# evalf/nutils

Measured on AMD Instinct MI355X. Metric: elements assembled/sec (global stiffness K), higher is better.
Workload: dtype f64; 1 GPU; 3D Poisson stiffness, 128^3 structured hex, p=1, 2x2x2 Gauss, iso geometry (BASELINE.json configs[1]); nelems_per_gpu=2097152, nnz_per_gpu=57066625, kernel=k_p1hex_skew<16,16,false,false>, parallelism=single GPU, launch=hipGraph replay (20 steps per graph), settle_steps=600

## Files before the change

nutils_amd/csrc/nh_p1hex_element.inc:

```
        double X[2][2][2][3];
        double un[8];
#pragma unroll
        for (int a = 0; a < 2; ++a)
#pragma unroll
          for (int bb = 0; bb < 2; ++bb)
#pragma unroll
            for (int c = 0; c < 2; ++c) {
              const double *src = NH_P1HEX_VERT(a, bb, c);
              X[a][bb][c][0] = src[0];
              X[a][bb][c][1] = src[1];
              X[a][bb][c][2] = src[2];
              un[a * 4 + bb * 2 + c] = VEC ? src[VW - 1] : 0.;
            }
#define NH_P1HEX_ELEM (((i64)gi * p.n1 + gj) * p.n2 + gk)
        double qs[8];
#pragma unroll
        for (int q = 0; q < 8; ++q) qs[q] = 1.;
        if (COEF && p.qscale) {
          const double *src = p.qscale + NH_P1HEX_ELEM * 8;
#pragma unroll
          for (int q = 0; q < 8; ++q) qs[q] = src[q];
        }
        constexpr bool hasm = MASS;
        double qm[8];
#pragma unroll
        for (int q = 0; q < 8; ++q) qm[q] = 1.;
        if (MASS && COEF && p.qmass) {
          const double *src = p.qmass + NH_P1HEX_ELEM * 8;
#pragma unroll
          for (int q = 0; q < 8; ++q) qm[q] = src[q];
        }
        double *const pl[2] = {acc + slot_of(gi) + (ej * VK + ek) * NS, acc + slot_of(gi + 1) + (ej * VK + ek) * NS};
#define NH_P1HEX_SLOT(a0, a1, a2, b0, b1, b2) (pl[a0] + ((a1) * VK + (a2)) * NS + ((b0) - (a0)) * 9 + ((b1) - (a1)) * 3 + ((b2) - (a2)))
        if constexpr (VEC) {
          double r[8];
#define NH_P1HEX_QS(q) qs[q]
#define NH_P1HEX_QM(q) qm[q]
#include "nh_p1hex_apply.inc"
#undef NH_P1HEX_QS
#undef NH_P1HEX_QM
#pragma unroll
          for (int a = 0; a < 8; ++a) atomicAdd(NH_P1HEX_SLOT(a >> 2, (a >> 1) & 1, a & 1, a >> 2, (a >> 1) & 1, a & 1), r[a]);
        } else {
        double R0[3][3], R1[3][3], R2[3][3], W01[2][2][3], W02[2][2][3], W12[2][2][3], Mm[3][3][3];
#define NH_P1HEX_QS(q) qs[q]
#define NH_P1HEX_QM(q) qm[q]
#include "nh_p1hex_math.inc"
#undef NH_P1HEX_QS
#undef NH_P1HEX_QM
        auto entry = [&](int a, int bb) {
          const int a0 = a >> 2, a1 = (a >> 1) & 1, a2 = a & 1;
          const int b0 = bb >> 2, b1 = (bb >> 1) & 1, b2 = bb & 1;
          const int p0 = a0 + b0, p1 = a1 + b1, p2 = a2 + b2;
          const double s00 = (a0 == b0) ? 1. : -1., s11 = (a1 == b1) ? 1. : -1., s22 = (a2 == b2) ? 1. : -1.;
          const double s01 = (a0 == b1) ? 1. : -1., s10 = (b0 == a1) ? 1. : -1.;
          const double s02 = (a0 == b2) ? 1. : -1., s20 = (b0 == a2) ? 1. : -1.;
          const double s12 = (a1 == b2) ? 1. : -1., s21 = (b1 == a2) ? 1. : -1.;
          double k = s00 * R0[p1][p2] + s11 * R1[p0][p2] + s22 * R2[p0][p1] + s01 * W01[b0][a1][p2] + s10 * W01[a0][b1][p2]
                   + s02 * W02[b0][a2][p1] + s20 * W02[a0][b2][p1] + s12 * W12[b1][a2][p0] + s21 * W12[a1][b2][p0];
          if (hasm) k += Mm[p0][p1][p2];
          return k;
        };
        {
#pragma unroll
          for (int a = 0; a < 8; ++a) {
            const int a0 = a >> 2, a1 = (a >> 1) & 1, a2 = a & 1;
#pragma unroll
            for (int bb = a; bb < 8; ++bb) {
              const int b0 = bb >> 2, b1 = (bb >> 1) & 1, b2 = bb & 1;
              const double k = entry(a, bb);
              double *const dst = NH_P1HEX_SLOT(a0, a1, a2, b0, b1, b2);
              if (!(DEBUG(p) & 1)) atomicAdd(dst, k);
              else if (k == 1.2345e300) dst[0] = 1.;
            }
          }
        }
        }
#undef NH_P1HEX_ELEM
#undef NH_P1HEX_SLOT
```

nutils_amd/csrc/nh_p1hex_math.inc:

```
{
  const double (&n)[2][2] = p.n;
  const double (&c)[3][2] = p.c;
  double J0[2][2][3], J1[2][2][3], J2[2][2][3];
#pragma unroll
  for (int d = 0; d < 3; ++d) {
    double e0[2][2], e1[2][2], e2[2][2];
#pragma unroll
    for (int x = 0; x < 2; ++x)
#pragma unroll
      for (int y = 0; y < 2; ++y) {
        e0[x][y] = X[1][x][y][d] - X[0][x][y][d];
        e1[x][y] = X[x][1][y][d] - X[x][0][y][d];
        e2[x][y] = X[x][y][1][d] - X[x][y][0][d];
      }
    double t0[2][2], t1[2][2], t2[2][2];
#pragma unroll
    for (int y = 0; y < 2; ++y) {
      const double d0 = e0[1][y] - e0[0][y], d1 = e1[1][y] - e1[0][y], d2 = e2[1][y] - e2[0][y];
#pragma unroll
      for (int q1 = 0; q1 < 2; ++q1) {
        t0[q1][y] = fma(n[1][q1], d0, e0[0][y]);
        t1[q1][y] = fma(n[1][q1], d1, e1[0][y]);
        t2[q1][y] = fma(n[1][q1], d2, e2[0][y]);
      }
    }
#pragma unroll
    for (int q1 = 0; q1 < 2; ++q1) {
      const double d0 = t0[q1][1] - t0[q1][0], d1 = t1[q1][1] - t1[q1][0], d2 = t2[q1][1] - t2[q1][0];
#pragma unroll
      for (int q2 = 0; q2 < 2; ++q2) {
        J0[q1][q2][d] = fma(n[1][q2], d0, t0[q1][0]);
        J1[q1][q2][d] = fma(n[1][q2], d1, t1[q1][0]);
        J2[q1][q2][d] = fma(n[1][q2], d2, t2[q1][0]);
      }
    }
  }
  double D0[2][2], D1[2][2], D2[2][2], M01[2][2][2], M02[2][2][2], M12[2][2][2], Dm[2][2][2];
#pragma unroll
  for (int qa = 0; qa < 2; ++qa)
#pragma unroll
    for (int qb = 0; qb < 2; ++qb)
#pragma unroll
      for (int qc = 0; qc < 2; ++qc) {
        const double *c0 = J0[qb][qc], *c1 = J1[qa][qc], *c2 = J2[qa][qb];
        double A[3][3];
        A[0][0] = c1[1] * c2[2] - c1[2] * c2[1];
        A[0][1] = c1[2] * c2[0] - c1[0] * c2[2];
        A[0][2] = c1[0] * c2[1] - c1[1] * c2[0];
        A[1][0] = c2[1] * c0[2] - c2[2] * c0[1];
        A[1][1] = c2[2] * c0[0] - c2[0] * c0[2];
        A[1][2] = c2[0] * c0[1] - c2[1] * c0[0];
        A[2][0] = c0[1] * c1[2] - c0[2] * c1[1];
        A[2][1] = c0[2] * c1[0] - c0[0] * c1[2];
        A[2][2] = c0[0] * c1[1] - c0[1] * c1[0];
        const double det = c0[0] * A[0][0] + c0[1] * A[0][1] + c0[2] * A[0][2];
        const double sc = p.wk[qa][qb][qc] * NH_P1HEX_QS(qa * 4 + qb * 2 + qc) * fast_rcp(fabs(det));
        const double m00 = sc * (A[0][0] * A[0][0] + A[0][1] * A[0][1] + A[0][2] * A[0][2]);
        const double m11 = sc * (A[1][0] * A[1][0] + A[1][1] * A[1][1] + A[1][2] * A[1][2]);
        const double m22 = sc * (A[2][0] * A[2][0] + A[2][1] * A[2][1] + A[2][2] * A[2][2]);
        M01[qa][qb][qc] = sc * (A[0][0] * A[1][0] + A[0][1] * A[1][1] + A[0][2] * A[1][2]);
        M02[qa][qb][qc] = sc * (A[0][0] * A[2][0] + A[0][1] * A[2][1] + A[0][2] * A[2][2]);
        M12[qa][qb][qc] = sc * (A[1][0] * A[2][0] + A[1][1] * A[2][1] + A[1][2] * A[2][2]);
        D0[qb][qc] = qa ? D0[qb][qc] + m00 : m00;
        D1[qa][qc] = qb ? D1[qa][qc] + m11 : m11;
        D2[qa][qb] = qc ? D2[qa][qb] + m22 : m22;
        if (hasm) Dm[qa][qb][qc] = p.wm[qa][qb][qc] * NH_P1HEX_QM(qa * 4 + qb * 2 + qc) * fabs(det);
      }
  {
    double U[2][3];
#pragma unroll
    for (int x = 0; x < 2; ++x)
#pragma unroll
      for (int pp = 0; pp < 3; ++pp) U[x][pp] = c[pp][0] * D0[x][0] + c[pp][1] * D0[x][1];
#pragma unroll
    for (int p1 = 0; p1 < 3; ++p1)
#pragma unroll
      for (int p2 = 0; p2 < 3; ++p2) R0[p1][p2] = c[p1][0] * U[0][p2] + c[p1][1] * U[1][p2];
#pragma unroll
    for (int x = 0; x < 2; ++x)
#pragma unroll
      for (int pp = 0; pp < 3; ++pp) U[x][pp] = c[pp][0] * D1[x][0] + c[pp][1] * D1[x][1];
#pragma unroll
    for (int p0 = 0; p0 < 3; ++p0)
#pragma unroll
      for (int p2 = 0; p2 < 3; ++p2) R1[p0][p2] = c[p0][0] * U[0][p2] + c[p0][1] * U[1][p2];
#pragma unroll
    for (int x = 0; x < 2; ++x)
#pragma unroll
      for (int pp = 0; pp < 3; ++pp) U[x][pp] = c[pp][0] * D2[x][0] + c[pp][1] * D2[x][1];
#pragma unroll
    for (int p0 = 0; p0 < 3; ++p0)
#pragma unroll
      for (int p1 = 0; p1 < 3; ++p1) R2[p0][p1] = c[p0][0] * U[0][p1] + c[p0][1] * U[1][p1];
  }
  {
    double V[2][2][2], V2[2][2][2];
#pragma unroll
    for (int b0 = 0; b0 < 2; ++b0)
#pragma unroll
      for (int be = 0; be < 2; ++be)
#pragma unroll
        for (int ga = 0; ga < 2; ++ga) V[b0][be][ga] = n[b0][0] * M01[0][be][ga] + n[b0][1] * M01[1][be][ga];
#pragma unroll
    for (int b0 = 0; b0 < 2; ++b0)
#pragma unroll
      for (int a1 = 0; a1 < 2; ++a1)
#pragma unroll
        for (int ga = 0; ga < 2; ++ga) V2[b0][a1][ga] = n[a1][0] * V[b0][0][ga] + n[a1][1] * V[b0][1][ga];
#pragma unroll
    for (int b0 = 0; b0 < 2; ++b0)
#pragma unroll
      for (int a1 = 0; a1 < 2; ++a1)
#pragma unroll
        for (int pp = 0; pp < 3; ++pp) W01[b0][a1][pp] = c[pp][0] * V2[b0][a1][0] + c[pp][1] * V2[b0][a1][1];
#pragma unroll
    for (int b0 = 0; b0 < 2; ++b0)
#pragma unroll
      for (int be = 0; be < 2; ++be)
#pragma unroll
        for (int ga = 0; ga < 2; ++ga) V[b0][be][ga] = n[b0][0] * M02[0][be][ga] + n[b0][1] * M02[1][be][ga];
#pragma unroll
    for (int b0 = 0; b0 < 2; ++b0)
#pragma unroll
      for (int a2 = 0; a2 < 2; ++a2)
#pragma unroll
        for (int be = 0; be < 2; ++be) V2[b0][a2][be] = n[a2][0] * V[b0][be][0] + n[a2][1] * V[b0][be][1];
#pragma unroll
    for (int b0 = 0; b0 < 2; ++b0)
#pragma unroll
      for (int a2 = 0; a2 < 2; ++a2)
#pragma unroll
        for (int pp = 0; pp < 3; ++pp) W02[b0][a2][pp] = c[pp][0] * V2[b0][a2][0] + c[pp][1] * V2[b0][a2][1];
#pragma unroll
    for (int b1 = 0; b1 < 2; ++b1)
#pragma unroll
      for (int al = 0; al < 2; ++al)
#pragma unroll
        for (int ga = 0; ga < 2; ++ga) V[b1][al][ga] = n[b1][0] * M12[al][0][ga] + n[b1][1] * M12[al][1][ga];
#pragma unroll
    for (int b1 = 0; b1 < 2; ++b1)
#pragma unroll
      for (int a2 = 0; a2 < 2; ++a2)
#pragma unroll
        for (int al = 0; al < 2; ++al) V2[b1][a2][al] = n[a2][0] * V[b1][al][0] + n[a2][1] * V[b1][al][1];
#pragma unroll
    for (int b1 = 0; b1 < 2; ++b1)
#pragma unroll
      for (int a2 = 0; a2 < 2; ++a2)
#pragma unroll
        for (int pp = 0; pp < 3; ++pp) W12[b1][a2][pp] = c[pp][0] * V2[b1][a2][0] + c[pp][1] * V2[b1][a2][1];
  }
  if (hasm) {
    double t1[2][2][3], t2[2][3][3];
#pragma unroll
    for (int qa = 0; qa < 2; ++qa)
#pragma unroll
      for (int qb = 0; qb < 2; ++qb)
#pragma unroll
        for (int p2 = 0; p2 < 3; ++p2) t1[qa][qb][p2] = c[p2][0] * Dm[qa][qb][0] + c[p2][1] * Dm[qa][qb][1];
#pragma unroll
    for (int qa = 0; qa < 2; ++qa)
#pragma unroll
      for (int p1 = 0; p1 < 3; ++p1)
#pragma unroll
        for (int p2 = 0; p2 < 3; ++p2) t2[qa][p1][p2] = c[p1][0] * t1[qa][0][p2] + c[p1][1] * t1[qa][1][p2];
#pragma unroll
    for (int p0 = 0; p0 < 3; ++p0)
#pragma unroll
      for (int p1 = 0; p1 < 3; ++p1)
#pragma unroll
        for (int p2 = 0; p2 < 3; ++p2) Mm[p0][p1][p2] = c[p0][0] * t2[0][p1][p2] + c[p0][1] * t2[1][p1][p2];
  }
}
```

Baseline: 11.91 billion elements/s.

## Factor P1 hex entry assembly, simplify Jacobian interpolation, inline reciprocal refinement

The per-entry loop that summed nine signed terms for each of the 36 upper-triangle stiffness entries is replaced by a staged evaluation per p0 slice. It precomputes shared sums S, P, Y01 and Y02 so common subexpressions are reused across entries. The Jacobian setup is rewritten as a trilinear coefficient form with fewer subtractions and FMAs. The reciprocal of the determinant now uses the hardware rcp estimate plus one inlined second-order refinement instead of fast_rcp. The aim is fewer FP64 instructions per element, at the cost of more intricate index logic and slightly different rounding.

```diff
diff --git a/nutils_amd/csrc/nh_p1hex_element.inc b/nutils_amd/csrc/nh_p1hex_element.inc
--- a/nutils_amd/csrc/nh_p1hex_element.inc
+++ b/nutils_amd/csrc/nh_p1hex_element.inc
@@ -48,33 +48,12 @@
 #include "nh_p1hex_math.inc"
 #undef NH_P1HEX_QS
 #undef NH_P1HEX_QM
-        auto entry = [&](int a, int bb) {
-          const int a0 = a >> 2, a1 = (a >> 1) & 1, a2 = a & 1;
-          const int b0 = bb >> 2, b1 = (bb >> 1) & 1, b2 = bb & 1;
-          const int p0 = a0 + b0, p1 = a1 + b1, p2 = a2 + b2;
-          const double s00 = (a0 == b0) ? 1. : -1., s11 = (a1 == b1) ? 1. : -1., s22 = (a2 == b2) ? 1. : -1.;
-          const double s01 = (a0 == b1) ? 1. : -1., s10 = (b0 == a1) ? 1. : -1.;
-          const double s02 = (a0 == b2) ? 1. : -1., s20 = (b0 == a2) ? 1. : -1.;
-          const double s12 = (a1 == b2) ? 1. : -1., s21 = (b1 == a2) ? 1. : -1.;
-          double k = s00 * R0[p1][p2] + s11 * R1[p0][p2] + s22 * R2[p0][p1] + s01 * W01[b0][a1][p2] + s10 * W01[a0][b1][p2]
-                   + s02 * W02[b0][a2][p1] + s20 * W02[a0][b2][p1] + s12 * W12[b1][a2][p0] + s21 * W12[a1][b2][p0];
-          if (hasm) k += Mm[p0][p1][p2];
-          return k;
-        };
-        {
-#pragma unroll
-          for (int a = 0; a < 8; ++a) {
-            const int a0 = a >> 2, a1 = (a >> 1) & 1, a2 = a & 1;
-#pragma unroll
-            for (int bb = a; bb < 8; ++bb) {
-              const int b0 = bb >> 2, b1 = (bb >> 1) & 1, b2 = bb & 1;
-              const double k = entry(a, bb);
-              double *const dst = NH_P1HEX_SLOT(a0, a1, a2, b0, b1, b2);
-              if (!(DEBUG(p) & 1)) atomicAdd(dst, k);
-              else if (k == 1.2345e300) dst[0] = 1.;
-            }
-          }
-        }
+#define NH_P1HEX_ENTRY(a0, a1, a2, b0, b1, b2, k) { \
+          double *const dst = NH_P1HEX_SLOT(a0, a1, a2, b0, b1, b2); \
+          if (!(DEBUG(p) & 1)) atomicAdd(dst, k); \
+          else if (k == 1.2345e300) dst[0] = 1.; }
+#include "nh_p1hex_entries.inc"
+#undef NH_P1HEX_ENTRY
         }
 #undef NH_P1HEX_ELEM
 #undef NH_P1HEX_SLOT
diff --git a/nutils_amd/csrc/nh_p1hex_entries.inc b/nutils_amd/csrc/nh_p1hex_entries.inc
--- /dev/null
+++ b/nutils_amd/csrc/nh_p1hex_entries.inc
@@ -0,0 +1,44 @@
+#pragma unroll
+for (int p0 = 0; p0 < 3; ++p0) {
+  const int a0 = p0 == 2, b0 = p0 >= 1;
+  double S[3][3], P[4][4], Y01[2][2][3], Y02[2][2][3];
+#pragma unroll
+  for (int p1 = 0; p1 < 3; ++p1)
+#pragma unroll
+    for (int p2 = 0; p2 < 3; ++p2) {
+      double s = (p0 == 1 ? -R0[p1][p2] : R0[p1][p2]) + (p1 == 1 ? -R1[p0][p2] : R1[p0][p2]);
+      s += p2 == 1 ? -R2[p0][p1] : R2[p0][p1];
+      if (hasm) s += Mm[p0][p1][p2];
+      S[p1][p2] = s;
+    }
+#pragma unroll
+  for (int u = 0; u < 4; ++u)
+#pragma unroll
+    for (int v = u; v < 4; ++v) {
+      const int x = u >> 1, y = u & 1, z = v >> 1, w = v & 1;
+      if (u == v) P[u][v] = fma(x == y ? 2. : -2., W12[x][y][p0], S[2 * x][2 * y]);
+      else P[u][v] = (S[x + z][y + w] + (x == w ? W12[z][y][p0] : -W12[z][y][p0])) + (z == y ? W12[x][w][p0] : -W12[x][w][p0]);
+    }
+#pragma unroll
+  for (int y = 0; y < 2; ++y)
+#pragma unroll
+    for (int w = (a0 == b0 ? y + 1 : 0); w < 2; ++w)
+#pragma unroll
+      for (int pp = 0; pp < 3; ++pp) {
+        const int x = a0, z = b0;
+        Y01[y][w][pp] = (x == w ? W01[z][y][pp] : -W01[z][y][pp]) + (z == y ? W01[x][w][pp] : -W01[x][w][pp]);
+        Y02[y][w][pp] = (x == w ? W02[z][y][pp] : -W02[z][y][pp]) + (z == y ? W02[x][w][pp] : -W02[x][w][pp]);
+      }
+#pragma unroll
+  for (int u = 0; u < 4; ++u)
+#pragma unroll
+    for (int v = (a0 == b0 ? u : 0); v < 4; ++v) {
+      const int a1 = u >> 1, a2 = u & 1, b1 = v >> 1, b2 = v & 1, p1 = a1 + b1, p2 = a2 + b2;
+      double k = P[u < v ? u : v][u < v ? v : u];
+      if (a0 == b0 && a1 == b1) k = fma(a0 == a1 ? 2. : -2., W01[a0][a1][p2], k);
+      else k += Y01[a1][b1][p2];
+      if (a0 == b0 && a2 == b2) k = fma(a0 == a2 ? 2. : -2., W02[a0][a2][p1], k);
+      else k += Y02[a0 == b0 && a2 > b2 ? b2 : a2][a0 == b0 && a2 > b2 ? a2 : b2][p1];
+      NH_P1HEX_ENTRY(a0, a1, a2, b0, b1, b2, k)
+    }
+}
diff --git a/nutils_amd/csrc/nh_p1hex_math.inc b/nutils_amd/csrc/nh_p1hex_math.inc
--- a/nutils_amd/csrc/nh_p1hex_math.inc
+++ b/nutils_amd/csrc/nh_p1hex_math.inc
@@ -1,39 +1,33 @@
+#ifndef NH_P1HEX_RCP_EST
+#define NH_P1HEX_RCP_EST(d) __builtin_amdgcn_rcp(d)
+#endif
 {
   const double (&n)[2][2] = p.n;
   const double (&c)[3][2] = p.c;
   double J0[2][2][3], J1[2][2][3], J2[2][2][3];
 #pragma unroll
   for (int d = 0; d < 3; ++d) {
-    double e0[2][2], e1[2][2], e2[2][2];
+    const double a0 = X[1][0][0][d] - X[0][0][0][d], a1 = X[0][1][0][d] - X[0][0][0][d], a2 = X[0][0][1][d] - X[0][0][0][d];
+    const double f02 = X[1][0][1][d] - X[0][0][1][d];
+    const double a01 = (X[1][1][0][d] - X[0][1][0][d]) - a0, a02 = f02 - a0, a12 = (X[0][1][1][d] - X[0][0][1][d]) - a1;
+    const double a012 = ((X[1][1][1][d] - X[0][1][1][d]) - f02) - a01;
+    double u0[2], v0[2], u1[2], u2[2], v12[2];
 #pragma unroll
-    for (int x = 0; x < 2; ++x)
-#pragma unroll
-      for (int y = 0; y < 2; ++y) {
-        e0[x][y] = X[1][x][y][d] - X[0][x][y][d];
-        e1[x][y] = X[x][1][y][d] - X[x][0][y][d];
-        e2[x][y] = X[x][y][1][d] - X[x][y][0][d];
-      }
-    double t0[2][2], t1[2][2], t2[2][2];
-#pragma unroll
-    for (int y = 0; y < 2; ++y) {
-      const double d0 = e0[1][y] - e0[0][y], d1 = e1[1][y] - e1[0][y], d2 = e2[1][y] - e2[0][y];
-#pragma unroll
-      for (int q1 = 0; q1 < 2; ++q1) {
-        t0[q1][y] = fma(n[1][q1], d0, e0[0][y]);
-        t1[q1][y] = fma(n[1][q1], d1, e1[0][y]);
-        t2[q1][y] = fma(n[1][q1], d2, e2[0][y]);
-      }
+    for (int q = 0; q < 2; ++q) {
+      u0[q] = fma(n[1][q], a01, a0);
+      v0[q] = fma(n[1][q], a012, a02);
+      u1[q] = fma(n[1][q], a01, a1);
+      u2[q] = fma(n[1][q], a02, a2);
+      v12[q] = fma(n[1][q], a012, a12);
     }
 #pragma unroll
-    for (int q1 = 0; q1 < 2; ++q1) {
-      const double d0 = t0[q1][1] - t0[q1][0], d1 = t1[q1][1] - t1[q1][0], d2 = t2[q1][1] - t2[q1][0];
+    for (int q1 = 0; q1 < 2; ++q1)
 #pragma unroll
       for (int q2 = 0; q2 < 2; ++q2) {
-        J0[q1][q2][d] = fma(n[1][q2], d0, t0[q1][0]);
-        J1[q1][q2][d] = fma(n[1][q2], d1, t1[q1][0]);
-        J2[q1][q2][d] = fma(n[1][q2], d2, t2[q1][0]);
+        J0[q1][q2][d] = fma(n[1][q2], v0[q1], u0[q1]);
+        J1[q1][q2][d] = fma(n[1][q2], v12[q1], u1[q1]);
+        J2[q1][q2][d] = fma(n[1][q2], v12[q1], u2[q1]);
       }
-    }
   }
   double D0[2][2], D1[2][2], D2[2][2], M01[2][2][2], M02[2][2][2], M12[2][2][2], Dm[2][2][2];
 #pragma unroll
@@ -54,7 +48,8 @@
         A[2][1] = c0[2] * c1[0] - c0[0] * c1[2];
         A[2][2] = c0[0] * c1[1] - c0[1] * c1[0];
         const double det = c0[0] * A[0][0] + c0[1] * A[0][1] + c0[2] * A[0][2];
-        const double sc = p.wk[qa][qb][qc] * NH_P1HEX_QS(qa * 4 + qb * 2 + qc) * fast_rcp(fabs(det));
+        const double ad = fabs(det), r = NH_P1HEX_RCP_EST(ad), e = fma(-ad, r, 1.), sr = p.wk[qa][qb][qc] * NH_P1HEX_QS(qa * 4 + qb * 2 + qc) * r;
+        const double sc = fma(sr, fma(e, e, e), sr);
         const double m00 = sc * (A[0][0] * A[0][0] + A[0][1] * A[0][1] + A[0][2] * A[0][2]);
         const double m11 = sc * (A[1][0] * A[1][0] + A[1][1] * A[1][1] + A[1][2] * A[1][2]);
         const double m22 = sc * (A[2][0] * A[2][0] + A[2][1] * A[2][1] + A[2][2] * A[2][2]);
```

New measurement: 11.73 billion elements/s. 0.985x the previous value.
